# ansonb/RECON

Hardware: AMD Instinct MI355X
Metric: edges aggregated/sec (GAT fwd+bwd) on synthetic KG-context graphs (higher is better)
Workload: dtype f32

## Files before the change

### recon_amd/csrc/gat_atp.hip

```cpp
#include <math.h>
#include <stdlib.h>
#include "recon_common.h"

#include <type_traits>

namespace recon {
namespace {

constexpr int kBlock = 256;

__device__ __forceinline__ int xcd_block(int b, int nb) {
    const int q = nb >> 3, r = nb & 7, x = b & 7, i = b >> 3;
    return (x < r ? x * (q + 1) : r * (q + 1) + (x - r) * q) + i;
}
template <int VEC, bool B16>
__device__ __forceinline__ void load_in(float (&r)[VEC], const float* base, int64_t e) {
    if constexpr (!B16) {
        load_vec<VEC>(r, base + e);
    } else {
        const uint16_t* b = reinterpret_cast<const uint16_t*>(base) + e;
        if constexpr (VEC == 4) {
            const uint2 t = *reinterpret_cast<const uint2*>(b);
            r[0] = __builtin_bit_cast(float, t.x << 16); r[1] = __builtin_bit_cast(float, t.x & 0xffff0000u);
            r[2] = __builtin_bit_cast(float, t.y << 16); r[3] = __builtin_bit_cast(float, t.y & 0xffff0000u);
// ... 1948 lines not shown
    if (rc != RECON_OK) return rc;
    rc = recon_gat_atp_aggregate(g, a, stream);
    if (rc != RECON_OK) return rc;
    return recon_gat_atp_project(g, a, stream);
}

extern "C" int recon_gat_atp_bwd_gee_bf16_supported(int32_t F, int32_t R, int32_t D, int32_t H) {
    recon::AtpShape s;
    if (!recon_gat_atp_bf16_io_supported(F, R, D, H) || !recon::atp_shape(F, R, H, &s)) return 0;
    const size_t lds_k2 = static_cast<size_t>(H) * (F + R) * sizeof(float) + (kBlock / 64) * 512;
    const bool lring = s.vec == 4 && s.kr == 1 && lds_k2 + (kBlock / 64) * kK2LdsRingBytes <= 64 * 1024 && cfg_char(CFG_K2_LDS_RING) != '0';
    return (s.ht >= H && lring) ? 1 : 0;
}

extern "C" size_t recon_gat_atp_bwd_split_bytes(int32_t N, int32_t D, int32_t H) {
    if (N <= 0 || D <= 0 || H <= 0) return 256;
    return align_up(static_cast<size_t>(3) * N * bx3_kp(H * D) * 2, 256);
}

extern "C" size_t recon_gat_atp_bwd_partial_floats(int32_t N, int32_t E, int32_t F, int32_t R, int32_t D, int32_t H) {
    const int64_t W = 2LL * F + R;
    int s1 = gemm_pick_split_k(static_cast<int32_t>(W), D, N, H);
    const int s2 = bx3_kmajor_splits(N, bx3_kmajor_split_k(static_cast<int32_t>(W), D, N, H));
    if (s2 > s1) s1 = s2;
    size_t need = static_cast<size_t>(s1) * H * D * W;
    (void)E; (void)F; (void)R;
    return need > 0 ? need : 1;
}

constexpr int kSkinnySlices = 1024;
constexpr size_t kSkinnySrcLdsMax = 32 * 1024;
static int skinny_rpb(int64_t rows) {
    const int rpb = static_cast<int>(ceil_div64(rows, kSkinnySlices));
    return rpb < 32 ? 32 : rpb;
}
extern "C" size_t recon_gat_atp_bwd_partial2_floats(int32_t N, int32_t E, int32_t F, int32_t R, int32_t D, int32_t H) {
    (void)N; (void)E; (void)D; (void)H;
    const size_t mx = static_cast<size_t>(F > R ? F : R);
    return static_cast<size_t>(3) * kSkinnySlices * 16 * mx;
}
static int32_t skinny_red_blocks(int nj, int K) { return static_cast<int32_t>(ceil_div64(1LL * nj * K, 16)); }

extern "C" int recon_gat_atp_bwd_ride_plan(int32_t NR, int32_t N, int32_t E, int32_t F, int32_t R, int32_t D, int32_t H, int32_t* plan) {
    if (!plan || NR < 0 || N < 1 || E < 0 || F < 1 || R < 1 || D < 1 || H < 1) return 0;
    const int64_t rows[3] = {NR, N, E};
    const int K[3] = {F, F, R};
    int32_t nr_total = 0;
    for (int i = 0; i < 3; ++i) {
        plan[i] = rows[i] > 0 ? static_cast<int32_t>(ceil_div64(rows[i], skinny_rpb(rows[i]))) : 0;
        plan[3 + i] = rows[i] > 0 ? skinny_red_blocks(H, K[i]) : 0;
        nr_total += plan[3 + i];
    }
    const int32_t W = 2 * F + R;
    const int sk = bx3_kmajor_splits(NR, bx3_kmajor_split_k(W, D, NR, H));
    const int64_t tiles_xy = hx2_kmajor_tiles_xy(W, D);
    plan[6] = sk;
    plan[7] = static_cast<int32_t>(tiles_xy * H * sk);
    plan[8] = static_cast<int32_t>(1LL * H * sk + hx2_kmajor_rider_layers(tiles_xy, nr_total));
    plan[9] = nr_total;
    const bool lds_ok = static_cast<size_t>(skinny_rpb(N)) * H * sizeof(float) <= kSkinnySrcLdsMax;
    return (H <= 8 && D <= 256 && lds_ok && recon_gat_atp_f16x2_supported(F, R, D, H) && nr_total > 0) ? 1 : 0;
}

extern "C" int recon_gat_atp_bwd(const recon_graph* g, const recon_gat_atp_bwd_args* b, recon_stream_t stream) {
    return recon_gat_atp_bwd_phase(g, b, RECON_ATP_BWD_ALL, stream);
}

extern "C" int recon_gat_atp_bwd_phase(const recon_graph* g, const recon_gat_atp_bwd_args* b, int32_t phases, recon_stream_t stream) {
    if (!b) return RECON_ERR_INVALID;
    const recon_gat_atp_args* a = &b->fwd;
    int rc = check_atp(g, a);
    if (rc != RECON_OK) return rc;
    if (!recon_gat_atp_supported(a->N, a->E, a->F, a->R, a->D, a->H)) return RECON_ERR_UNSUPPORTED;
    if (!a->Z || !a->Zk || !b->grad_out || !b->g_V || !b->gxd || !b->Gs || !b->g_u || !b->partial || !b->partial2 || !b->q) return RECON_ERR_INVALID;
    if (a->E > 0 && (!a->sigma || !b->g_sigma || !b->Gxs)) return RECON_ERR_INVALID;
    const bool hx2 = atp_hx2(a);
    if ((a->concat || atp_rows(g, a).row_node) && !b->g_h && !hx2) return RECON_ERR_INVALID;
    if (hx2 && (!b->gh_split || (reinterpret_cast<uintptr_t>(b->gh_split) & 15) || (b->ld_gout & 3))) return RECON_ERR_INVALID;
    if (b->ld_gout < a->H * a->D) return RECON_ERR_INVALID;
    if (a->N == 0) return RECON_OK;
    hipStream_t st = as_stream(stream);
    const int32_t N = a->N, E = a->E, F = a->F, R = a->R, D = a->D, H = a->H, W = 2 * F + R;
    const AtpRows rw = atp_rows(g, a);
    const int32_t NR = rw.n;
    const int64_t HD = 1LL * H * D;
    AtpShape s;
    atp_shape(F, R, H, &s);
    const size_t lds_u = static_cast<size_t>(H) * (F + R) * sizeof(float);
    if (lds_u > 60 * 1024) return RECON_ERR_UNSUPPORTED;
    const size_t lds_k2 = lds_u + (kBlock / 64) * 512;

    const float* gh = b->grad_out;
    int32_t ld_gh = b->ld_gout;
    const int64_t ld_ghp = bx3_kp(static_cast<int32_t>(HD));
    const bool gh_planes = hx2 || (b->gh_split && a->a_split && !(reinterpret_cast<uintptr_t>(b->gh_split) & 15) && (D % 8) == 0 &&
                                   ((b->ld_gout | a->ld_out) & 3) == 0);
    uint16_t* ghp = gh_planes ? static_cast<uint16_t*>(b->gh_split) : nullptr;
    const int64_t ldi = (static_cast<int64_t>(NR) + 7) / 8 * 8;
    const size_t inv_off = align_up(static_cast<size_t>(2) * N * bx3_kp(static_cast<int32_t>(HD)) * 2, 256);
    const bool row_scaled = hx2 && D <= 256 && ((a->ld_out | b->ld_gout) & 3) == 0 && cfg_char(CFG_ATP_ROW_SCALE) != '0' &&
                            inv_off + static_cast<size_t>(H) * ldi * sizeof(float) <= recon_gat_atp_bwd_split_bytes(N, D, H);
    float* row_inv = row_scaled ? reinterpret_cast<float*>(static_cast<char*>(b->gh_split) + inv_off) : nullptr;
    if (phases & RECON_ATP_BWD_PREPARE) {
        if (hx2 && !row_scaled) {
            rc = hx2_amax(b->grad_out, N, static_cast<int32_t>(HD), b->ld_gout, atp_q(a, 3), st);
            if (rc != RECON_OK) return rc;
        }
// ... 108 lines not shown
                for (int i = 0; i < 3; ++i) {
                    sj[i] = SkinnyJob{nullptr, nullptr, nullptr, nullptr, 0, 0, 0, 0, 1, 0};
                    rj[i] = SkinnyRedJob{nullptr, nullptr, 0, 0, 0, 0, 0, 1, 0};
                    if (i >= count) continue;
                    const Prod& q = pr[i];
                    if (q.rows <= 0) {
                        for (int j = 0; j < q.nj; ++j) (void)hipMemsetAsync(q.out + (j % q.P) * q.S1 + (j / q.P) * q.S2, 0, sizeof(float) * q.K, st);
                        continue;
                    }
                    const int rpb = skinny_rpb(q.rows);
                    const int nb = static_cast<int>(ceil_div64(q.rows, rpb));
                    float* part = b->partial2 + i * third;
                    sj[i] = SkinnyJob{q.G, q.X, q.gather, part, q.ldg, q.nj, q.rows, q.K, rpb, nb};
                    rj[i] = SkinnyRedJob{part, q.out, q.S1, q.S2, nb, q.nj, q.K, q.P, skinny_red_blocks(q.nj, q.K)};
                    if (q.nj > nj_max) nj_max = q.nj;
                    nb_total += nb; nr_total += rj[i].nblocks;
                }
                if (share) { launch_src(); if (nb_total == 0) return; }
                else {
                    if (nb_total == 0) return;
                    const dim3 gp(static_cast<unsigned>(nb_total));
                    if (a->io_bf16) {
                        if (nj_max <= 8) hipLaunchKernelGGL((k_skinny_tn_partial<8, true>), gp, dim3(256), 0, st, sj[0], sj[1], sj[2]);
                        else hipLaunchKernelGGL((k_skinny_tn_partial<16, true>), gp, dim3(256), 0, st, sj[0], sj[1], sj[2]);
                    } else if (nj_max <= 8) hipLaunchKernelGGL((k_skinny_tn_partial<8>), gp, dim3(256), 0, st, sj[0], sj[1], sj[2]);
                    else hipLaunchKernelGGL((k_skinny_tn_partial<16>), gp, dim3(256), 0, st, sj[0], sj[1], sj[2]);
                }
                if (ride) { rider.j[0] = rj[0]; rider.j[1] = rj[1]; rider.j[2] = rj[2]; rider.nblocks = nr_total; }
                else hipLaunchKernelGGL(k_skinny_reduce, dim3(static_cast<unsigned>(nr_total)), dim3(1024), 0, st, rj[0], rj[1], rj[2]);
            };
            if (H <= 8) {
                const Prod pr[3] = {{b->Gs, 2 * H, H, a->x, rw.row_node, NR, F, H, W, 0, b->g_u},
                                    {b->Gs + H, 2 * H, H, a->x, nullptr, N, F, H, W, 0, b->g_u + F},
                                    {b->g_sigma, H, H, a->edge_embed, ee_gather, E, R, H, W, 0, b->g_u + 2 * F}};
                run_jobs(pr, 3);
            } else {
                for (int j = 0; j < 2 * H; ++j) {
                    const Prod one = {b->Gs + j, 2 * H, 1, a->x, j < H ? rw.row_node : nullptr, j < H ? NR : N, F, 1, W, 0,
                                      b->g_u + static_cast<int64_t>(j % H) * W + (j / H) * F};
                    run_jobs(&one, 1);
                }
                for (int h0 = 0; h0 < H; h0 += 16) {
                    const int nh = H - h0 < 16 ? H - h0 : 16;
                    const Prod one = {b->g_sigma + h0, H, nh, a->edge_embed, ee_gather, E, R, nh, W, 0, b->g_u + static_cast<int64_t>(h0) * W + 2 * F};
                    run_jobs(&one, 1);
                }
            }
        }
        RECON_CHECK_LAUNCH();
    }
    }
    if (b->g_a || b->g_a_2) {
        if (!b->g_a) return RECON_ERR_INVALID;
        if (phases & RECON_ATP_BWD_WEIGHTS) {
            OperandDesc A = plain_operand(a->V, static_cast<int64_t>(H) * W);
            OperandDesc B = plain_operand(gh, ld_gh);
            OutputDesc C = plain_output(b->g_a, W);
            GemmBatch bw = bt;
            bw.a_bs = W; bw.b_bs = D; bw.c_bs = static_cast<int64_t>(D) * W; bw.c_transpose = 1;
            const int64_t ldv = static_cast<int64_t>(H) * W;
            if (hx2) {
                const int sk = bx3_kmajor_splits(NR, bx3_kmajor_split_k(W, D, NR, H));
                rc = gemm_hx2_kmajor_batched(W, D, NR, a->V, 2LL * W, W, 2LL * NR * W, b->gh_split, 2LL * D, D, 2LL * NR * D,
                                             H, sk, b->partial, static_cast<const char*>(a->aux) + kHx2ZeroPageOffset, atp_scale_v(a), atp_scale_g(a), st,
                                             atp_dst_shared(a), row_inv, ldi, rider.nblocks > 0 ? &rider : nullptr);
                if (rc == RECON_OK && (phases & RECON_ATP_BWD_EARLY_SUM)) rc = splitk_reduce(b->partial, sk, W, D, C, bw.c_bs, H, 0, true, st);
            } else if (gh_planes && bx3_kmajor_supported(a->V, ldv, W, ld_ghp, D, W, D)) {
                const int sk = bx3_kmajor_splits(NR, bx3_kmajor_split_k(W, D, NR, H));
                rc = gemm_bx3_kmajor_batched(W, D, NR, a->V, ldv, W, b->gh_split, ld_ghp, static_cast<int64_t>(NR) * ld_ghp, D, H, sk, b->partial, st);
                if (rc == RECON_OK) rc = splitk_reduce(b->partial, sk, W, D, C, bw.c_bs, H, 0, true, st);
            } else {
                const int sk = gemm_pick_split_k(W, D, NR, H);
                rc = gemm_f32_batched(W, D, NR, A, false, B, false, C, bw, sk, b->partial, st);
            }
            if (rc != RECON_OK) return rc;
        }
        if ((phases & RECON_ATP_BWD_FINISH) && hx2 && !(phases & RECON_ATP_BWD_EARLY_SUM)) {
            const int sk = bx3_kmajor_splits(NR, bx3_kmajor_split_k(W, D, NR, H));
            const int ntile = static_cast<int>(ceil_div64(W, 32) * ceil_div64(D, 32)) * H;
            hipLaunchKernelGGL(k_atp_weights_finish, dim3(static_cast<unsigned>(ntile + ceil_div64(1LL * H * D, 8))), dim3(256), 0, st, b->partial, sk, W,
                               D, H, a->a, a->a_2, b->g_u, b->g_a, b->g_a_2, atp_q(a, 3), kHx2QuantityWords);
        } else if (phases & RECON_ATP_BWD_FINISH)
        hipLaunchKernelGGL(k_score_vec_bwd, dim3(static_cast<unsigned>(D), static_cast<unsigned>(H)), dim3(256), 0, st, a->a, a->a_2, b->g_u,
                           D, W, b->g_a, b->g_a_2, atp_hx2(a) ? atp_q(a, 3) : nullptr, kHx2QuantityWords);
        RECON_CHECK_LAUNCH();
    } else if ((phases & RECON_ATP_BWD_FINISH) && atp_hx2(a)) {
        if (hipMemsetAsync(atp_q(a, 3), 0, sizeof(uint32_t) * kHx2QuantityWords, st) != hipSuccess) return RECON_ERR_LAUNCH;
    }
    return RECON_OK;
}
```

### recon_amd/csrc/gemm_hx2.hip

```cpp
#include <stdlib.h>
#include "gemm_tile16.h"

namespace recon {
namespace {

constexpr int T = 2;

struct Hx2Args {
    const _Float16* Ap; const _Float16* Bp;
    int64_t a_plane, a_row, a_bs;
    int64_t b_plane, b_row, b_bs;
    OutputDesc C;
    int64_t c_bs;
    int32_t M, N, K;
    int32_t epilogue, c_vec4, xcd_remap, c_plain;
    int32_t a_shared_k;
    Hx2Scale sa, sb;
    const float* row_inv; int64_t row_inv_bs;
    int32_t a_span_bytes;
};

struct Hx2Terms {
    using V = f16x8;
    static constexpr int T = 2, NP = 3;
// ... 327 lines not shown
    bool b_rot[2];
#pragma unroll
    for (int hh = 0; hh < 2; ++hh) {
        const int k = 8 * g + 4 * hh + (ip >> 2);
#pragma unroll
        for (int i = 0; i < 2; ++i) a_off[i][hh] = k * 256 + (((2 * wid + i) ^ ka_h(k)) << 5) + ((ip & 3) << 3);
        b_row[hh] = k * (KB_SLOTS * 16) + (((ip & 3) & 1) << 3);
        b_rot[hh] = (k & 8) != 0;
    }
    auto b_off = [&](int j, int hh) { return b_row[hh] + (2 * j + ((ip & 3) >> 1) + (b_rot[hh] ? 2 : 0)) * 16; };
    float4 kin[2];
    float sg = 1.f;
    auto load_kinv = [&](int k0) {
        if constexpr (KSC) {
            const float* q = p.k_inv + bz * p.k_inv_bs + min(k0 + 8 * g, ((p.K + 7) & ~7) - 8);
            kin[0] = *reinterpret_cast<const float4*>(q);
            kin[1] = *reinterpret_cast<const float4*>(q + 4);
        }
    };
    auto mma_tile = [&]() {
        f16x8 a[2][T];
#pragma unroll
        for (int i = 0; i < 2; ++i)
#pragma unroll
            for (int q = 0; q < T; ++q) a[i][q] = tr_frag<f16x8>(As + q * KA_PLANE, a_off[i][0], a_off[i][1]);
        if constexpr (KSC) {
            const float f[8] = {kin[0].x, kin[0].y, kin[0].z, kin[0].w, kin[1].x, kin[1].y, kin[1].z, kin[1].w};
            f16x8 kf;
#pragma unroll
            for (int e = 0; e < 8; ++e) kf[e] = static_cast<_Float16>(fminf(f[e] * sg, 1.f));
#pragma unroll
            for (int i = 0; i < 2; ++i)
#pragma unroll
                for (int q = 0; q < T; ++q) a[i][q] = a[i][q] * kf;
        }
        mma_pairs<Hx2Terms>(acc, a, [&](int j, f16x8 (&dst)[T]) {
            const int o0 = b_off(j, 0), o1 = b_off(j, 1);
#pragma unroll
            for (int q = 0; q < T; ++q) dst[q] = tr_frag<f16x8>(Bs + q * KB_PLANE, o0, o1);
        });
    };

    if (k_begin < k_end) { dma(k_begin); load_kinv(k_begin); }
    const float ia = hx2_inv(hx2_scale_wave(p.sa));
    sg = hx2_scale_wave(p.sb);
    const float ib = hx2_inv(sg);
    for (int k0 = k_begin; k0 < k_end; k0 += BK) {
        asm volatile("s_waitcnt vmcnt(0)" ::: "memory");
        __syncthreads();
        mma_tile();
        __syncthreads();
        if (k0 + BK < k_end) { dma(k0 + BK); load_kinv(k0 + BK); }
    }
    float* base = p.partial + static_cast<int64_t>(tile.z) * p.M * p.N;
    const __amdgpu_buffer_rsrc_t rsrc = __builtin_amdgcn_make_buffer_rsrc(base, 0, p.M * p.N * 4, 0x00020000);
    const float sc = ia * ib;
#pragma unroll
    for (int i = 0; i < 2; ++i)
#pragma unroll
        for (int r = 0; r < 4; ++r) {
            const int row = m0 + mb + 16 * i + 4 * g + r;
            const int rowoff = row < p.M ? row * p.N : 0x1ffffff0;
#pragma unroll
            for (int j = 0; j < TN; ++j) {
                const int col = n0 + 16 * j + ip;
                const int off = col < p.N ? (rowoff + col) * 4 : 0x7ffffff0;
                __builtin_amdgcn_raw_buffer_store_b32(__builtin_bit_cast(uint32_t, acc[i][j][r] * sc), rsrc, off, 0, 0);
            }
        }
}

template <bool TRANS>
__global__ void __launch_bounds__(256) k_hx2_split_planes(const float* __restrict__ src, int64_t ld, int64_t src_bs, int32_t rows, int32_t K,
                                                          int32_t Kp, _Float16* __restrict__ dst, int64_t plane, int64_t dst_bs, const Hx2Scale sc) {
    const int64_t idx = static_cast<int64_t>(blockIdx.x) * 256 + threadIdx.x;
    const int kq = static_cast<int>(idx % (Kp / 8));
    const int r = static_cast<int>(idx / (Kp / 8));
    if (r >= rows) return;
    const float s = hx2_scale(sc);
    const float* sp = src + blockIdx.y * src_bs;
    float v[8];
#pragma unroll
    for (int j = 0; j < 8; ++j) {
        const int k = 8 * kq + j;
        v[j] = k < K ? (TRANS ? sp[static_cast<int64_t>(k) * ld + r] : sp[static_cast<int64_t>(r) * ld + k]) : 0.f;
    }
    uint32_t lo[4], hi[4];
#pragma unroll
    for (int j = 0; j < 4; ++j) hx2_split2(v[2 * j] * s, v[2 * j + 1] * s, lo[j], hi[j]);
    _Float16* d = dst + blockIdx.y * dst_bs + static_cast<int64_t>(r) * Kp + 8 * kq;
    *reinterpret_cast<u32x4*>(d) = u32x4{lo[0], lo[1], lo[2], lo[3]};
    *reinterpret_cast<u32x4*>(d + plane) = u32x4{hi[0], hi[1], hi[2], hi[3]};
}

__global__ void __launch_bounds__(256) k_hx2_split_both(const Hx2SplitBoth p) { hx2_split_both_block(p, blockIdx.x, blockIdx.y, blockIdx.z); }

template <int NTHREADS>
__global__ void __launch_bounds__(NTHREADS) k_hx2_amax(const float* __restrict__ src, int64_t rows, int32_t cols, int64_t ld, uint32_t* __restrict__ slot) {
    float m = 0.f;
    const int64_t stride = static_cast<int64_t>(gridDim.x) * NTHREADS;
    if (ld == cols && !(reinterpret_cast<uintptr_t>(src) & 15)) {
        const int64_t n = rows * cols, n4 = n >> 2;
        const float4* s4 = reinterpret_cast<const float4*>(src);
        int64_t i = static_cast<int64_t>(blockIdx.x) * NTHREADS + threadIdx.x;
        for (; i + 3 * stride < n4; i += 4 * stride) {
            const float4 v0 = s4[i], v1 = s4[i + stride], v2 = s4[i + 2 * stride], v3 = s4[i + 3 * stride];
// ... 72 lines not shown
    return RECON_OK;
}

bool hx2_supported(const void* Ap, int64_t a_plane, int64_t a_row, int64_t a_bs, int32_t K) {
    if (K <= 0 || (K & 7)) return false;
    return !((reinterpret_cast<uintptr_t>(Ap) & 15) || (a_plane & 7) || (a_row & 7) || (a_bs & 7));
}

int gemm_hx2_batched(int32_t M, int32_t N, int32_t K, const void* Ap, int64_t a_plane, int64_t a_row, int64_t a_bs, const void* Bplanes,
                     const OutputDesc& C, const GemmBatch& bt, const Hx2Scale& sa, const Hx2Scale& sb, hipStream_t st, int32_t a_shared_k,
                     const float* row_inv, int64_t row_inv_bs) {
    if (M < 0 || N < 0 || K < 0 || bt.batch < 0) return RECON_ERR_INVALID;
    if (M == 0 || N == 0 || bt.batch == 0) return RECON_OK;
    if (!Ap || !Bplanes || !C.base) return RECON_ERR_INVALID;
    if (!hx2_supported(Ap, a_plane, a_row, a_bs, K) || bt.c_transpose || bt.batch > 65535 || (reinterpret_cast<uintptr_t>(Bplanes) & 15))
        return RECON_ERR_UNSUPPORTED;
    Hx2Args a;
    a.Ap = static_cast<const _Float16*>(Ap); a.a_plane = a_plane; a.a_row = a_row; a.a_bs = a_bs;
    const int32_t Kp = hx2_kp(K);
    a.Bp = static_cast<const _Float16*>(Bplanes);
    a.b_row = Kp;
    a.b_bs = static_cast<int64_t>(N) * Kp;
    a.b_plane = a.b_bs * bt.batch;
    if (T * a.b_plane >= (1LL << 31)) return RECON_ERR_UNSUPPORTED;
    a.C = C; a.c_bs = bt.c_bs; a.M = M; a.N = N; a.K = K; a.epilogue = bt.epilogue;
    a.c_vec4 = c_vec4_ok(C, N, bt.c_bs) ? 1 : 0;
    a.xcd_remap = 1;
    if (a_shared_k < 0 || (a_shared_k & 7) || (a_shared_k && a_bs * bt.batch >= (1LL << 31))) return RECON_ERR_INVALID;
    a.a_shared_k = a_shared_k;
    a.c_plain = (a.c_vec4 && !C.scatter && C.P >= M && C.Dseg >= N && (static_cast<int64_t>(M) * C.S1 + N) * 4 < (1LL << 31)) ? 1 : 0;
    a.sa = sa; a.sb = sb;
    a.row_inv = row_inv; a.row_inv_bs = row_inv_bs;
    if (row_inv && sa.p0) return RECON_ERR_INVALID;
    const bool wide = K >= 1024 && ceil_div64(M, 256) * ceil_div64(N, BN) * bt.batch >= 256;
    const dim3 grid(static_cast<unsigned>(ceil_div64(N, BN)), static_cast<unsigned>(ceil_div64(M, wide ? 256 : BM)), static_cast<unsigned>(bt.batch));
    const int64_t a_span = ((T - 1) * a_plane + (bt.batch - 1) * a_bs + static_cast<int64_t>(M - 1) * a_row + hx2_kp(K) + 8) * 2;
    a.a_span_bytes = (a_plane >= 0 && a_bs >= 0 && a_row >= 0 && a_span < (1LL << 31) - 64) ? static_cast<int32_t>(a_span) : 0;
    const bool ring = !wide && a.a_span_bytes > 0 && cfg_char(CFG_HX2_RING) != '0';
    if (wide) hipLaunchKernelGGL((k_gemm_hx2<8>), grid, dim3(512), 0, st, a);
    else if (ring) hipLaunchKernelGGL((k_gemm_hx2_r3<4>), grid, dim3(NT), 0, st, a);
    else hipLaunchKernelGGL((k_gemm_hx2<4>), grid, dim3(NT), 0, st, a);
    if (hipGetLastError() != hipSuccess) return RECON_ERR_LAUNCH;
    return RECON_OK;
}

bool hx2_kmajor_supported(const void* Ap, int64_t lda, int64_t a_plane, int64_t a_bs, const void* Bp, int64_t ldb, int64_t b_plane,
                          int64_t b_bs, int32_t M, int32_t N) {
    const int64_t m_ld = (static_cast<int64_t>(M) + 7) / 8 * 8, n_ld = (static_cast<int64_t>(N) + 7) / 8 * 8;
    if (M < 1 || N < 1 || ((lda | a_plane | a_bs | ldb | b_plane | b_bs) & 7) || m_ld > lda || n_ld > ldb) return false;
    if (((M & 7) && a_bs != 0) || ((N & 7) && b_bs != 0)) return false;
    return !((reinterpret_cast<uintptr_t>(Ap) | reinterpret_cast<uintptr_t>(Bp)) & 15);
}

int64_t hx2_kmajor_tiles_xy(int32_t M, int32_t N) { return ceil_div64(N, BN) * ceil_div64(M, BM); }
int64_t hx2_kmajor_rider_layers(int64_t tiles_xy, int32_t rider_blocks) {
    return rider_blocks > 0 && tiles_xy > 0 ? ceil_div64(rider_blocks, tiles_xy) : 0;
}

int gemm_hx2_kmajor_batched(int32_t M, int32_t N, int32_t K, const void* Ap, int64_t lda, int64_t a_plane, int64_t a_bs, const void* Bp,
                            int64_t ldb, int64_t b_plane, int64_t b_bs, int32_t batch, int32_t split_k, float* partial, const void* zeros,
                            const Hx2Scale& sa, const Hx2Scale& sb, hipStream_t st, int32_t a_shared_m, const float* k_inv, int64_t k_inv_bs,
                            const SkinnyRedRider* rider) {
    if (M < 0 || N < 0 || K < 0 || batch < 0 || split_k < 1) return RECON_ERR_INVALID;
    const bool ride = rider && rider->nblocks > 0;
    if (ride && (M == 0 || N == 0 || batch == 0 || !k_inv)) return RECON_ERR_INVALID;
    if (M == 0 || N == 0 || batch == 0) return RECON_OK;
    if (!Ap || !Bp || !partial || !zeros || (reinterpret_cast<uintptr_t>(zeros) & 15)) return RECON_ERR_INVALID;
    if (!hx2_kmajor_supported(Ap, lda, a_plane, a_bs, Bp, ldb, b_plane, b_bs, M, N)) return RECON_ERR_UNSUPPORTED;
    Hx2KmArgs a;
    a.Ap = static_cast<const _Float16*>(Ap); a.Bp = static_cast<const _Float16*>(Bp); a.zeros = static_cast<const _Float16*>(zeros);
    a.lda = lda; a.ldb = ldb; a.a_plane = a_plane; a.b_plane = b_plane; a.a_bs = a_bs; a.b_bs = b_bs;
    a.partial = partial; a.M = M; a.N = N; a.K = K;
    a.m_ld = (M + 7) / 8 * 8; a.n_ld = (N + 7) / 8 * 8;
    const SplitK sp = splitk_plan(K, split_k);
    a.k_per_split = sp.k_per_split;
    a.nsplit = sp.nsplit;
    if (a.nsplit != split_k) return RECON_ERR_INVALID;
    a.tiles_z = batch * split_k;
    const int64_t gz = static_cast<int64_t>(a.tiles_z) + (ride ? hx2_kmajor_rider_layers(hx2_kmajor_tiles_xy(M, N), rider->nblocks) : 0);
    if (gz > 65535 || hx2_kmajor_tiles_xy(M, N) * gz >= (1LL << 31)) return RECON_ERR_UNSUPPORTED;
    a.sa = sa; a.sb = sb;
    if (a_shared_m < 0 || (a_shared_m & 7)) return RECON_ERR_UNSUPPORTED;
    a.a_shared_m = a_shared_m;
    const dim3 grid(static_cast<unsigned>(ceil_div64(N, BN)), static_cast<unsigned>(ceil_div64(M, BM)), static_cast<unsigned>(gz));
    a.k_inv = k_inv; a.k_inv_bs = k_inv_bs;
    if (k_inv && ((k_inv_bs & 3) || k_inv_bs < ((K + 7) & ~7) || (reinterpret_cast<uintptr_t>(k_inv) & 15))) return RECON_ERR_UNSUPPORTED;
    SkinnyRedRider none;
    none.nblocks = 0;
    for (SkinnyRedJob& j : none.j) j = SkinnyRedJob{nullptr, nullptr, 0, 0, 0, 0, 0, 1, 0};
    if (ride) hipLaunchKernelGGL((k_gemm_hx2_kmajor<2, true, true>), grid, dim3(NT), 0, st, a, *rider);
    else if (k_inv) hipLaunchKernelGGL((k_gemm_hx2_kmajor<2, true, false>), grid, dim3(NT), 0, st, a, none);
    else hipLaunchKernelGGL((k_gemm_hx2_kmajor<2, false, false>), grid, dim3(NT), 0, st, a, none);
    if (hipGetLastError() != hipSuccess) return RECON_ERR_LAUNCH;
    return RECON_OK;
}

}

static constexpr size_t kHdr = (recon::kHx2AuxBytes + 255) / 256 * 256;
extern "C" size_t recon_hx2_aux_bytes(void) { return recon::kHx2AuxBytes; }
static size_t hx2_planes_bytes(int64_t rows, int32_t K) { return align_up(static_cast<size_t>(2) * rows * recon::hx2_kp(K) * 2, 256); }

extern "C" size_t recon_sgemm_hx2_workspace_bytes(int32_t M, int32_t N, int32_t K) {
    if (M <= 0 || N <= 0 || K <= 0) return kHdr;
    return kHdr + hx2_planes_bytes(M, K) + hx2_planes_bytes(N, K);
}

extern "C" int recon_sgemm_hx2(int32_t M, int32_t N, int32_t K, const float* A, int32_t lda, const float* B, int32_t ldb, float* C_,
                               int32_t ldc, void* workspace, recon_stream_t stream) {
    using namespace recon;
    if (M < 0 || N < 0 || K < 0) return RECON_ERR_INVALID;
    if (M == 0 || N == 0) return RECON_OK;
    if (!A || !B || !C_ || !workspace || (reinterpret_cast<uintptr_t>(workspace) & 255)) return RECON_ERR_INVALID;
    if (K & 7) return RECON_ERR_UNSUPPORTED;
    hipStream_t st = as_stream(stream);
    char* ws = static_cast<char*>(workspace);
    uint32_t* slots = reinterpret_cast<uint32_t*>(ws);
    if (hipMemsetAsync(ws, 0, kHdr, st) != hipSuccess) return RECON_ERR_LAUNCH;
    int rc = hx2_amax(A, M, K, lda, slots + 0, st);
    if (rc == RECON_OK) rc = hx2_amax(B, N, K, ldb, slots + kHx2QuantityWords, st);
    if (rc != RECON_OK) return rc;
    const Hx2Scale sa{slots + 0, nullptr, 1.f}, sb{slots + kHx2QuantityWords, nullptr, 1.f};
    char* ap = ws + kHdr;
    char* bp = ap + hx2_planes_bytes(M, K);
    rc = hx2_split_planes(A, lda, 0, false, M, K, 1, ap, sa, st);
    if (rc == RECON_OK) rc = hx2_split_planes(B, ldb, 0, false, N, K, 1, bp, sb, st);
    if (rc != RECON_OK) return rc;
    GemmBatch bt;
    bt.batch = 1; bt.a_bs = bt.b_bs = bt.c_bs = 0; bt.epilogue = GEMM_EPI_NONE;
    const int64_t Kp = hx2_kp(K);
    return gemm_hx2_batched(M, N, K, ap, static_cast<int64_t>(M) * Kp, Kp, 0, bp, plain_output(C_, ldc), bt, sa, sb, st);
}

extern "C" int recon_sgemm_hx2_presplit(int32_t M, int32_t N, int32_t K, float* C_, int32_t ldc, void* workspace, recon_stream_t stream) {
    using namespace recon;
    if (M <= 0 || N <= 0 || K <= 0 || (K & 7) || !C_ || !workspace) return RECON_ERR_INVALID;
    char* ws = static_cast<char*>(workspace);
    uint32_t* slots = reinterpret_cast<uint32_t*>(ws);
    const Hx2Scale sa{slots + 0, nullptr, 1.f}, sb{slots + kHx2QuantityWords, nullptr, 1.f};
    char* ap = ws + kHdr;
    char* bp = ap + hx2_planes_bytes(M, K);
    GemmBatch bt;
    bt.batch = 1; bt.a_bs = bt.b_bs = bt.c_bs = 0; bt.epilogue = GEMM_EPI_NONE;
    const int64_t Kp = hx2_kp(K);
    return gemm_hx2_batched(M, N, K, ap, static_cast<int64_t>(M) * Kp, Kp, 0, bp, plain_output(C_, ldc), bt, sa, sb, as_stream(stream));
}

extern "C" size_t recon_sgemm_hx2_tn_workspace_bytes(int32_t M, int32_t N, int32_t K) {
    using namespace recon;
    if (M <= 0 || N <= 0 || K <= 0) return kHdr;
    const int sk = bx3_kmajor_splits(K, bx3_kmajor_split_k(M, N, K, 1));
    return kHdr + hx2_planes_bytes(K, M) + hx2_planes_bytes(K, N) + static_cast<size_t>(sk) * M * N * sizeof(float) + 256;
}

static int hx2_tn(int32_t M, int32_t N, int32_t K, const float* A, int32_t lda, const float* B, int32_t ldb, float* C_, int32_t ldc,
                  void* workspace, bool split, recon_stream_t stream) {
    using namespace recon;
    if (M < 0 || N < 0 || K < 0) return RECON_ERR_INVALID;
    if (M == 0 || N == 0) return RECON_OK;
    if (!C_ || !workspace || (reinterpret_cast<uintptr_t>(workspace) & 255)) return RECON_ERR_INVALID;
    hipStream_t st = as_stream(stream);
    char* ws = static_cast<char*>(workspace);
    uint32_t* slots = reinterpret_cast<uint32_t*>(ws);
    const Hx2Scale sa{slots + 0, nullptr, 1.f}, sb{slots + kHx2QuantityWords, nullptr, 1.f};
    char* ap = ws + kHdr;
    char* bp = ap + hx2_planes_bytes(K, M);
    float* partial = reinterpret_cast<float*>(bp + hx2_planes_bytes(K, N));
    const int64_t Mp = hx2_kp(M), Np = hx2_kp(N);
    int rc = RECON_OK;
    if (split) {
        if (!A || !B) return RECON_ERR_INVALID;
        if (hipMemsetAsync(ws, 0, kHdr, st) != hipSuccess) return RECON_ERR_LAUNCH;
        rc = hx2_amax(A, K, M, lda, slots + 0, st);
        if (rc == RECON_OK) rc = hx2_amax(B, K, N, ldb, slots + kHx2QuantityWords, st);
        if (rc == RECON_OK) rc = hx2_split_planes(A, lda, 0, false, K, M, 1, ap, sa, st);
        if (rc == RECON_OK) rc = hx2_split_planes(B, ldb, 0, false, K, N, 1, bp, sb, st);
        if (rc != RECON_OK) return rc;
    }
    const int sk = bx3_kmajor_splits(K, bx3_kmajor_split_k(M, N, K, 1));
    rc = gemm_hx2_kmajor_batched(M, N, K, ap, Mp, static_cast<int64_t>(K) * Mp, 0, bp, Np, static_cast<int64_t>(K) * Np, 0, 1, sk, partial,
                                 ws + kHx2ZeroPageOffset, sa, sb, st);
    if (rc != RECON_OK) return rc;
    return splitk_reduce(partial, sk, M, N, plain_output(C_, ldc), 0, 1, GEMM_EPI_NONE, false, st);
}

extern "C" int recon_sgemm_hx2_tn(int32_t M, int32_t N, int32_t K, const float* A, int32_t lda, const float* B, int32_t ldb, float* C_,
                                  int32_t ldc, void* workspace, recon_stream_t stream) {
    return hx2_tn(M, N, K, A, lda, B, ldb, C_, ldc, workspace, true, stream);
}
extern "C" int recon_sgemm_hx2_tn_presplit(int32_t M, int32_t N, int32_t K, float* C_, int32_t ldc, void* workspace, recon_stream_t stream) {
    return hx2_tn(M, N, K, nullptr, 0, nullptr, 0, C_, ldc, workspace, false, stream);
}
```

### recon_amd/csrc/gemm_tile16.h

```cpp
#pragma once
#include "gemm_common.h"

namespace recon {

constexpr int BM = 128, BN = 208, BK = 32, NT = 256, TN = 13;
using bf16x8 = __attribute__((ext_vector_type(8))) __bf16;
using f16x8 = __attribute__((ext_vector_type(8))) _Float16;
using f32x4 = __attribute__((ext_vector_type(4))) float;
using u32x4 = __attribute__((ext_vector_type(4))) uint32_t;
using i16x4 = __attribute__((ext_vector_type(4))) short;

constexpr int B_PLANE = BN * 64;
constexpr int KB_SLOTS = 28;
constexpr int KA_PLANE = BK * 256, KB_PLANE = BK * KB_SLOTS * 16;


__device__ __forceinline__ int lds_off(int row, int kq) { return row * 64 + (((kq + 2 * (row >> 3)) & 3) << 4); }

template <int T>
__device__ __forceinline__ int b_image_src(int slot, int n0, int N, int64_t b_plane, int64_t b_row) {
    const int s = min(slot, T * B_PLANE / 16 - 1);
    const int plane = T == 1 ? 0 : s / (BN * 4), rem = T == 1 ? s : s % (BN * 4), rowL = rem >> 2, pslot = rem & 3;
    const int kq = (pslot - 2 * (rowL >> 3)) & 3;
    const int j = rowL >> 4, rho = rowL & 15;
// ... 35 lines not shown
                        *reinterpret_cast<float4*>(crow + minor_off(C.Dseg, C.Sseg, col)) =
                            make_float4(fin(acc[i][4 * q][r]), fin(acc[i][4 * q + 1][r]), fin(acc[i][4 * q + 2][r]), fin(acc[i][4 * q + 3][r]));
                } else {
#pragma unroll
                    for (int jj = 0; jj < 4; ++jj)
                        if (col + jj < N) crow[minor_off(C.Dseg, C.Sseg, col + jj)] = fin(acc[i][4 * q + jj][r]);
                }
            }
            const int col = n0 + 192 + li;
            if (col < N) crow[minor_off(C.Dseg, C.Sseg, col)] = fin(acc[i][12][r]);
        }
}


template <class S, int NJ>
__device__ __forceinline__ void products(f32x4 (&acc)[2][TN], const typename S::V (&a)[2][S::T], const typename S::V (&b)[2][S::T], int j0) {
#pragma unroll
    for (int t = 0; t < S::NP; ++t)
#pragma unroll
        for (int jj = 0; jj < NJ; ++jj)
#pragma unroll
            for (int i = 0; i < 2; ++i) acc[i][j0 + jj] = S::mfma(t, a[i], b[jj], acc[i][j0 + jj]);
}

template <class S, class Read>
__device__ __forceinline__ void mma_pairs(f32x4 (&acc)[2][TN], const typename S::V (&a)[2][S::T], Read read) {
    typename S::V b[2][2][S::T];
    auto read_pair = [&](int j0, typename S::V (&dst)[2][S::T]) {
#pragma unroll
        for (int jj = 0; jj < 2; ++jj)
            if (j0 + jj < TN) read(j0 + jj, dst[jj]);
    };
    read_pair(0, b[0]);
#pragma unroll
    for (int g = 0; g < (TN + 1) / 2; ++g) {
        if (2 * g + 2 < TN) read_pair(2 * g + 2, b[(g + 1) & 1]);
        __builtin_amdgcn_sched_barrier(0);
        if (2 * g + 1 < TN) products<S, 2>(acc, a, b[g & 1], 2 * g);
        else products<S, 1>(acc, a, b[g & 1], 2 * g);
        __builtin_amdgcn_sched_barrier(0);
    }
}


__device__ __forceinline__ int ka_h(int k) { return (k & 3) | (((k >> 3) & 1) << 2); }

template <class V>
__device__ __forceinline__ V tr_frag(const unsigned char* base, int off_lo, int off_hi) {
    const i16x4 lo = __builtin_amdgcn_ds_read_tr16_b64_v4i16((__attribute__((address_space(3))) i16x4*)(base + off_lo));
    const i16x4 hi = __builtin_amdgcn_ds_read_tr16_b64_v4i16((__attribute__((address_space(3))) i16x4*)(base + off_hi));
    return __builtin_bit_cast(V, __builtin_shufflevector(lo, hi, 0, 1, 2, 3, 4, 5, 6, 7));
}


inline int32_t tile_kp(int32_t K) { return (K + BK - 1) / BK * BK; }

struct SplitK { int32_t k_per_split, nsplit; };
inline SplitK splitk_plan(int32_t K, int32_t split_k) {
    int64_t kps = ceil_div64(K > 0 ? K : 1, split_k);
    kps = ceil_div64(kps, BK) * BK;
    return {static_cast<int32_t>(kps), static_cast<int32_t>(ceil_div64(K > 0 ? K : 1, kps))};
}

inline bool c_vec4_ok(const OutputDesc& C, int32_t N, int64_t c_bs) {
    return !(N & 3) && !(c_bs & 3) && !(reinterpret_cast<uintptr_t>(C.base) & 15) && !(C.S1 & 3) && !(C.S2 & 3) && !(C.Sseg & 3) &&
           (C.Dseg >= N || !(C.Dseg & 3));
}

}
```

### recon_amd/csrc/recon_common.h

```cpp
#pragma once
#include <hip/hip_runtime.h>
#include <stdint.h>
#include "recon_hip.h"

#define RECON_CHECK_LAUNCH()                                   \
    do {                                                       \
        if (hipGetLastError() != hipSuccess) return RECON_ERR_LAUNCH; \
    } while (0)

static inline hipStream_t as_stream(recon_stream_t s) { return reinterpret_cast<hipStream_t>(s); }
static inline int64_t ceil_div64(int64_t a, int64_t b) { return (a + b - 1) / b; }
static inline size_t align_up(size_t x, size_t a) { return (x + a - 1) / a * a; }

namespace recon {

constexpr int kWave = 64;

enum CfgKey { CFG_GCN_FUSED, CFG_GCN_FUSED_BWD, CFG_GEMM_CFG, CFG_GEMM_LIN, CFG_GEMM_SPLITK, CFG_GEMM_XCD, CFG_PROP_B16, CFG_PROP_B16_YPOST,
              CFG_PROP_BWD, CFG_PROP_BWD_CHAIN, CFG_PROP_BWD_WIDE, CFG_PROP_FWD, CFG_PROP_LDS_KB, CFG_ATP_ROW_SCALE, CFG_GRAPH_SMALL, CFG_KG_NHOP,
              CFG_HX2_RING, CFG_K2_LDS_RING, CFG_K2_PERSIST, CFG_COUNT };
const char* cfg(CfgKey k);
int cfg_int(CfgKey k, int dflt);
char cfg_char(CfgKey k);
int32_t* nan_flag();
// ... 285 lines not shown
bool hx2_kmajor_supported(const void* Ap, int64_t lda, int64_t a_plane, int64_t a_bs, const void* Bp, int64_t ldb, int64_t b_plane,
                          int64_t b_bs, int32_t M, int32_t N);

struct SkinnyRedJob { const float* partial; float* out; int64_t S1, S2; int32_t nb, nj, K, P, nblocks; };
struct SkinnyRedRider { SkinnyRedJob j[3]; int32_t nblocks; };
template <int NT>
__device__ __forceinline__ void skinny_reduce_block(const SkinnyRedJob& j0, const SkinnyRedJob& j1, const SkinnyRedJob& j2, int blk, int tid,
                                                    float (*red)[17]) {
    static_assert(NT == 1024 || NT == 256, "64 slice groups x 16 elements over the block");
    constexpr int GPT = 1024 / NT, GSTEP = NT / 16;
    const int which = blk < j0.nblocks ? 0 : (blk < j0.nblocks + j1.nblocks ? 1 : 2);
    const SkinnyRedJob& jb = which == 0 ? j0 : (which == 1 ? j1 : j2);
    const float* __restrict__ partial = jb.partial;
    const int nb = jb.nb, tot = jb.nj * jb.K;
    const int bid = blk - (which == 0 ? 0 : (which == 1 ? j0.nblocks : j0.nblocks + j1.nblocks));
    const int e = tid & 15, g0 = tid >> 4;
    const int idx = bid * 16 + e;
    const int idc = min(idx, tot - 1);
    const int per = (nb + 63) / 64;
    float s[GPT][4];
    int b0[GPT], len[GPT];
#pragma unroll
    for (int i = 0; i < GPT; ++i) {
        b0[i] = (g0 + i * GSTEP) * per;
        len[i] = max(0, min(nb, b0[i] + per) - b0[i]);
        s[i][0] = s[i][1] = s[i][2] = s[i][3] = 0.f;
    }
    for (int k = 0; k < per; k += 4) {
        float v[GPT][4];
#pragma unroll
        for (int i = 0; i < GPT; ++i)
#pragma unroll
            for (int q = 0; q < 4; ++q) v[i][q] = partial[static_cast<int64_t>(min(b0[i] + k + q, nb - 1)) * tot + idc];
#pragma unroll
        for (int i = 0; i < GPT; ++i) {
            const bool quad = k + 4 <= len[i];
#pragma unroll
            for (int q = 0; q < 4; ++q) s[i][q] = quad ? s[i][q] + v[i][q] : s[i][q];
#pragma unroll
            for (int q = 0; q < 4; ++q) s[i][0] = (!quad && k + q < len[i]) ? s[i][0] + v[i][q] : s[i][0];
        }
    }
#pragma unroll
    for (int i = 0; i < GPT; ++i) red[g0 + i * GSTEP][e] = (s[i][0] + s[i][1]) + (s[i][2] + s[i][3]);
    __syncthreads();
    if (g0 == 0 && idx < tot) {
        float t = 0.f;
#pragma unroll
        for (int g = 0; g < 64; ++g) t += red[g][e];
        const int j = idx / jb.K, c = idx % jb.K;
        jb.out[(j % jb.P) * jb.S1 + (j / jb.P) * jb.S2 + c] = t;
    }
}
int64_t hx2_kmajor_tiles_xy(int32_t M, int32_t N);
int64_t hx2_kmajor_rider_layers(int64_t tiles_xy, int32_t rider_blocks);
int gemm_hx2_kmajor_batched(int32_t M, int32_t N, int32_t K, const void* Ap, int64_t lda, int64_t a_plane, int64_t a_bs, const void* Bp,
                            int64_t ldb, int64_t b_plane, int64_t b_bs, int32_t batch, int32_t split_k, float* partial, const void* zeros,
                            const Hx2Scale& sa, const Hx2Scale& sb, hipStream_t st, int32_t a_shared_m = 0, const float* k_inv = nullptr,
                            int64_t k_inv_bs = 0, const SkinnyRedRider* rider = nullptr);
int splitk_reduce(const float* partial, int32_t splits, int32_t M, int32_t N, const OutputDesc& C, int64_t c_bs, int32_t batch,
                  int32_t epilogue, bool transpose, hipStream_t st);

}
```

Before: 82.52 million.

## Add 256-row wide-tile k-major hx2 GEMM kernel for standalone TN sgemm path

```diff
diff --git a/recon_amd/csrc/gat_atp.hip b/recon_amd/csrc/gat_atp.hip
--- a/recon_amd/csrc/gat_atp.hip
+++ b/recon_amd/csrc/gat_atp.hip
@@ -2024,7 +2024,7 @@
         nr_total += plan[3 + i];
     }
     const int32_t W = 2 * F + R;
-    const int sk = bx3_kmajor_splits(NR, bx3_kmajor_split_k(W, D, NR, H));
+    const int sk = bx3_kmajor_splits(NR, hx2_kmajor_split_k(W, D, NR, H, false));
     const int64_t tiles_xy = hx2_kmajor_tiles_xy(W, D);
     plan[6] = sk;
     plan[7] = static_cast<int32_t>(tiles_xy * H * sk);
@@ -2239,6 +2239,7 @@
     }
     if (b->g_a || b->g_a_2) {
         if (!b->g_a) return RECON_ERR_INVALID;
+        const int sk_hx2 = hx2 ? bx3_kmajor_splits(NR, hx2_kmajor_split_k(W, D, NR, H, false)) : 1;
         if (phases & RECON_ATP_BWD_WEIGHTS) {
             OperandDesc A = plain_operand(a->V, static_cast<int64_t>(H) * W);
             OperandDesc B = plain_operand(gh, ld_gh);
@@ -2247,7 +2248,7 @@
             bw.a_bs = W; bw.b_bs = D; bw.c_bs = static_cast<int64_t>(D) * W; bw.c_transpose = 1;
             const int64_t ldv = static_cast<int64_t>(H) * W;
             if (hx2) {
-                const int sk = bx3_kmajor_splits(NR, bx3_kmajor_split_k(W, D, NR, H));
+                const int sk = sk_hx2;
                 rc = gemm_hx2_kmajor_batched(W, D, NR, a->V, 2LL * W, W, 2LL * NR * W, b->gh_split, 2LL * D, D, 2LL * NR * D,
                                              H, sk, b->partial, static_cast<const char*>(a->aux) + kHx2ZeroPageOffset, atp_scale_v(a), atp_scale_g(a), st,
                                              atp_dst_shared(a), row_inv, ldi, rider.nblocks > 0 ? &rider : nullptr);
@@ -2263,7 +2264,7 @@
             if (rc != RECON_OK) return rc;
         }
         if ((phases & RECON_ATP_BWD_FINISH) && hx2 && !(phases & RECON_ATP_BWD_EARLY_SUM)) {
-            const int sk = bx3_kmajor_splits(NR, bx3_kmajor_split_k(W, D, NR, H));
+            const int sk = sk_hx2;
             const int ntile = static_cast<int>(ceil_div64(W, 32) * ceil_div64(D, 32)) * H;
             hipLaunchKernelGGL(k_atp_weights_finish, dim3(static_cast<unsigned>(ntile + ceil_div64(1LL * H * D, 8))), dim3(256), 0, st, b->partial, sk, W,
                                D, H, a->a, a->a_2, b->g_u, b->g_a, b->g_a_2, atp_q(a, 3), kHx2QuantityWords);
diff --git a/recon_amd/csrc/gemm_hx2.hip b/recon_amd/csrc/gemm_hx2.hip
--- a/recon_amd/csrc/gemm_hx2.hip
+++ b/recon_amd/csrc/gemm_hx2.hip
@@ -403,6 +403,164 @@
         __syncthreads();
         if (k0 + BK < k_end) { dma(k0 + BK); load_kinv(k0 + BK); }
     }
+    float* base = p.partial + static_cast<int64_t>(tile.z) * p.M * p.N;
+    const __amdgpu_buffer_rsrc_t rsrc = __builtin_amdgcn_make_buffer_rsrc(base, 0, p.M * p.N * 4, 0x00020000);
+    const float sc = ia * ib;
+#pragma unroll
+    for (int i = 0; i < 2; ++i)
+#pragma unroll
+        for (int r = 0; r < 4; ++r) {
+            const int row = m0 + mb + 16 * i + 4 * g + r;
+            const int rowoff = row < p.M ? row * p.N : 0x1ffffff0;
+#pragma unroll
+            for (int j = 0; j < TN; ++j) {
+                const int col = n0 + 16 * j + ip;
+                const int off = col < p.N ? (rowoff + col) * 4 : 0x7ffffff0;
+                __builtin_amdgcn_raw_buffer_store_b32(__builtin_bit_cast(uint32_t, acc[i][j][r] * sc), rsrc, off, 0, 0);
+            }
+        }
+}
+
+constexpr int KA256_PIECES = T * (KA256_PLANE / 1024), KA256_DMA = KA256_PIECES / 8;
+constexpr int KB256_DMA = (KB_PIECES + 7) / 8;
+constexpr int KM256_A_RING = 3, KM256_A_STAGE = T * KA256_PLANE, KM256_B_STAGE = T * KB_PLANE;
+constexpr int KM256_B_AT = KM256_A_RING * KM256_A_STAGE, KM256_SCRATCH_AT = KM256_B_AT + 2 * KM256_B_STAGE;
+constexpr int KM256_LDS = KM256_SCRATCH_AT + 1024;
+
+__global__ void __launch_bounds__(512, 1) k_gemm_hx2_kmajor256(const Hx2KmArgs p) {
+    __shared__ __attribute__((aligned(16))) unsigned char S[KM256_LDS];
+    unsigned char* const scratch = S + KM256_SCRATCH_AT;
+    const int t = threadIdx.x, lane = t & 63;
+    const int wid = __builtin_amdgcn_readfirstlane(t >> 6);
+    const TileId tile = xcd_tile(1);
+    const int m0 = tile.y * BM256, n0 = tile.x * BN;
+    const int bz = tile.z / p.nsplit, zs = tile.z % p.nsplit;
+    const int k_begin = zs * p.k_per_split, k_end = min(p.K, k_begin + p.k_per_split);
+    const int KT = k_begin < k_end ? (k_end - k_begin + BK - 1) / BK : 0;
+
+    const _Float16* pa[KA256_DMA];
+    const _Float16* pb[KB256_DMA];
+    int a_k[KA256_DMA], b_k[KB256_DMA];
+#pragma unroll
+    for (int i = 0; i < KA256_DMA; ++i) {
+        const int pc = 8 * i + wid, s = 64 * (pc & 15) + lane;
+        a_k[i] = k_begin + (s >> 5);
+        int64_t col = min(m0 + ka256_src_col(s), p.m_ld - 8);
+        if (col >= p.a_shared_m) col += bz * p.a_bs;
+        pa[i] = p.Ap + (pc >> 4) * p.a_plane + static_cast<int64_t>(a_k[i]) * p.lda + col;
+    }
+#pragma unroll
+    for (int i = 0; i < KB256_DMA; ++i) {
+        const int pc = min(8 * i + wid, KB_PIECES - 1);
+        const int s = 64 * (pc % (KB_PIECES / T)) + lane, k = s / KB_SLOTS, phys = s % KB_SLOTS;
+        int slot = phys - ((k & 8) ? 2 : 0);
+        if (slot < 0 || slot >= 26) slot = 0;
+        b_k[i] = k_begin + k;
+        pb[i] = p.Bp + bz * p.b_bs + (pc / (KB_PIECES / T)) * p.b_plane + static_cast<int64_t>(b_k[i]) * p.ldb + min(n0 + 8 * slot, p.n_ld - 8);
+    }
+    const _Float16* zlane = p.zeros + 8 * lane;
+    const int64_t a_step = static_cast<int64_t>(BK) * p.lda, b_step = static_cast<int64_t>(BK) * p.ldb;
+    int ka_adv = 0, kb_adv = 0;
+    auto dma_a = [&](int stage) {
+        const bool real = k_begin + ka_adv < k_end;
+        unsigned char* const st = S + stage * KM256_A_STAGE;
+#pragma unroll
+        for (int i = 0; i < KA256_DMA; ++i) {
+            const int pc = 8 * i + wid;
+            dma16_to_lds(a_k[i] + ka_adv < k_end ? pa[i] : zlane, real ? st + (pc >> 4) * KA256_PLANE + 1024 * (pc & 15) : scratch);
+            pa[i] += a_step;
+        }
+        ka_adv += BK;
+    };
+    auto dma_b = [&](int stage) {
+        const bool real = k_begin + kb_adv < k_end;
+        unsigned char* const st = S + KM256_B_AT + stage * KM256_B_STAGE;
+#pragma unroll
+        for (int i = 0; i < KB256_DMA; ++i) {
+            const int pc = 8 * i + wid;
+            const bool piece = real && pc < KB_PIECES;
+            dma16_to_lds(b_k[i] + kb_adv < k_end ? pb[i] : zlane, piece ? st + (pc / (KB_PIECES / T)) * KB_PLANE + 1024 * (pc % (KB_PIECES / T)) : scratch);
+            pb[i] += b_step;
+        }
+        kb_adv += BK;
+    };
+
+    f32x4 acc[2][TN];
+#pragma unroll
+    for (int i = 0; i < 2; ++i)
+#pragma unroll
+        for (int j = 0; j < TN; ++j) acc[i][j] = f32x4{0.f, 0.f, 0.f, 0.f};
+
+    const int mb = wid * 32;
+    const int ip = lane & 15, g = lane >> 4;
+    int a_off[2][2], b_base[2];
+#pragma unroll
+    for (int hh = 0; hh < 2; ++hh) {
+        const int k = 8 * g + 4 * hh + (ip >> 2);
+#pragma unroll
+        for (int i = 0; i < 2; ++i) a_off[i][hh] = ka256_off(k, 2 * wid + i, ip);
+        b_base[hh] = k * (KB_SLOTS * 16) + (((ip & 3) & 1) << 3) + ((((ip & 3) >> 1) + ((k & 8) ? 2 : 0)) << 4);
+    }
+    int sa = 0, par = 0;
+    auto step = [&]() {
+        dma_wait<KA256_DMA>();
+        __builtin_amdgcn_s_barrier();
+        asm volatile("" ::: "memory");
+        const unsigned char* At = S + sa * KM256_A_STAGE;
+        const unsigned char* Bt = S + KM256_B_AT + par * KM256_B_STAGE;
+        const int sa_free = sa == 0 ? KM256_A_RING - 1 : sa - 1;
+        sa = sa + 1 == KM256_A_RING ? 0 : sa + 1;
+        par ^= 1;
+        f16x8 a[2][T];
+#pragma unroll
+        for (int i = 0; i < 2; ++i)
+#pragma unroll
+            for (int q = 0; q < T; ++q) a[i][q] = tr_frag<f16x8>(At + q * KA256_PLANE, a_off[i][0], a_off[i][1]);
+        f16x8 b[2][2][T];
+        auto read_pair = [&](int j0, f16x8 (&dst)[2][T]) {
+#pragma unroll
+            for (int jj = 0; jj < 2; ++jj)
+                if (j0 + jj < TN) {
+#pragma unroll
+                    for (int q = 0; q < T; ++q) dst[jj][q] = tr_frag<f16x8>(Bt + q * KB_PLANE, b_base[0] + (j0 + jj) * 32, b_base[1] + (j0 + jj) * 32);
+                }
+        };
+        read_pair(0, b[0]);
+#pragma unroll
+        for (int gq = 0; gq < (TN + 1) / 2; ++gq) {
+            if (2 * gq + 2 < TN) read_pair(2 * gq + 2, b[(gq + 1) & 1]);
+            __builtin_amdgcn_sched_barrier(0);
+            if (2 * gq + 1 < TN) products<Hx2Terms, 2>(acc, a, b[gq & 1], 2 * gq);
+            else products<Hx2Terms, 1>(acc, a, b[gq & 1], 2 * gq);
+            __builtin_amdgcn_sched_barrier(0);
+            if (gq == 0) {
+                dma_b(par);
+                dma_a(sa_free);
+                __builtin_amdgcn_sched_barrier(0);
+            }
+        }
+    };
+
+    dma_a(0);
+    dma_b(0);
+    dma_a(1);
+    const float ia = hx2_inv(hx2_scale_wave(p.sa)), ib = hx2_inv(hx2_scale_wave(p.sb));
+    const bool live = m0 + mb < p.M;
+    if (live) {
+#pragma unroll 1
+        for (int kt = 0; kt < KT; ++kt) step();
+    } else {
+#pragma unroll 1
+        for (int kt = 0; kt < KT; ++kt) {
+            dma_wait<KA256_DMA>();
+            __builtin_amdgcn_s_barrier();
+            asm volatile("" ::: "memory");
+            dma_b((kt + 1) & 1);
+            dma_a((kt + 2) % KM256_A_RING);
+        }
+    }
+    dma_wait<0>();
+    if (!live) return;
     float* base = p.partial + static_cast<int64_t>(tile.z) * p.M * p.N;
     const __amdgpu_buffer_rsrc_t rsrc = __builtin_amdgcn_make_buffer_rsrc(base, 0, p.M * p.N * 4, 0x00020000);
     const float sc = ia * ib;
@@ -581,7 +739,16 @@
     return !((reinterpret_cast<uintptr_t>(Ap) | reinterpret_cast<uintptr_t>(Bp)) & 15);
 }
 
-int64_t hx2_kmajor_tiles_xy(int32_t M, int32_t N) { return ceil_div64(N, BN) * ceil_div64(M, BM); }
+bool hx2_kmajor_wide(int32_t M, bool wide) { return wide && M > BM; }
+int64_t hx2_kmajor_tiles_xy(int32_t M, int32_t N, bool wide) { return ceil_div64(N, BN) * ceil_div64(M, hx2_kmajor_wide(M, wide) ? BM256 : BM); }
+int hx2_kmajor_split_k(int32_t M, int32_t N, int32_t K, int32_t batch, bool wide) {
+    if (!hx2_kmajor_wide(M, wide)) return bx3_kmajor_split_k(M, N, K, batch);
+    const int64_t tiles = hx2_kmajor_tiles_xy(M, N, true) * (batch > 0 ? batch : 1);
+    int64_t s = 256 / (tiles > 0 ? tiles : 1);
+    if (s > K / (4 * BK)) s = K / (4 * BK);
+    if (s > 64) s = 64;
+    return static_cast<int>(s < 1 ? 1 : s);
+}
 int64_t hx2_kmajor_rider_layers(int64_t tiles_xy, int32_t rider_blocks) {
     return rider_blocks > 0 && tiles_xy > 0 ? ceil_div64(rider_blocks, tiles_xy) : 0;
 }
@@ -589,7 +756,7 @@
 int gemm_hx2_kmajor_batched(int32_t M, int32_t N, int32_t K, const void* Ap, int64_t lda, int64_t a_plane, int64_t a_bs, const void* Bp,
                             int64_t ldb, int64_t b_plane, int64_t b_bs, int32_t batch, int32_t split_k, float* partial, const void* zeros,
                             const Hx2Scale& sa, const Hx2Scale& sb, hipStream_t st, int32_t a_shared_m, const float* k_inv, int64_t k_inv_bs,
-                            const SkinnyRedRider* rider) {
+                            const SkinnyRedRider* rider, bool want_wide) {
     if (M < 0 || N < 0 || K < 0 || batch < 0 || split_k < 1) return RECON_ERR_INVALID;
     const bool ride = rider && rider->nblocks > 0;
     if (ride && (M == 0 || N == 0 || batch == 0 || !k_inv)) return RECON_ERR_INVALID;
@@ -606,18 +773,21 @@
     a.nsplit = sp.nsplit;
     if (a.nsplit != split_k) return RECON_ERR_INVALID;
     a.tiles_z = batch * split_k;
-    const int64_t gz = static_cast<int64_t>(a.tiles_z) + (ride ? hx2_kmajor_rider_layers(hx2_kmajor_tiles_xy(M, N), rider->nblocks) : 0);
-    if (gz > 65535 || hx2_kmajor_tiles_xy(M, N) * gz >= (1LL << 31)) return RECON_ERR_UNSUPPORTED;
+    const int64_t gz = static_cast<int64_t>(a.tiles_z) + (ride ? hx2_kmajor_rider_layers(hx2_kmajor_tiles_xy(M, N, want_wide), rider->nblocks) : 0);
+    if (gz > 65535 || hx2_kmajor_tiles_xy(M, N, want_wide) * gz >= (1LL << 31)) return RECON_ERR_UNSUPPORTED;
     a.sa = sa; a.sb = sb;
     if (a_shared_m < 0 || (a_shared_m & 7)) return RECON_ERR_UNSUPPORTED;
     a.a_shared_m = a_shared_m;
-    const dim3 grid(static_cast<unsigned>(ceil_div64(N, BN)), static_cast<unsigned>(ceil_div64(M, BM)), static_cast<unsigned>(gz));
+    const bool wide = hx2_kmajor_wide(M, want_wide);
+    if (wide && (ride || k_inv)) return RECON_ERR_UNSUPPORTED;
+    const dim3 grid(static_cast<unsigned>(ceil_div64(N, BN)), static_cast<unsigned>(ceil_div64(M, wide ? BM256 : BM)), static_cast<unsigned>(gz));
     a.k_inv = k_inv; a.k_inv_bs = k_inv_bs;
     if (k_inv && ((k_inv_bs & 3) || k_inv_bs < ((K + 7) & ~7) || (reinterpret_cast<uintptr_t>(k_inv) & 15))) return RECON_ERR_UNSUPPORTED;
     SkinnyRedRider none;
     none.nblocks = 0;
     for (SkinnyRedJob& j : none.j) j = SkinnyRedJob{nullptr, nullptr, 0, 0, 0, 0, 0, 1, 0};
-    if (ride) hipLaunchKernelGGL((k_gemm_hx2_kmajor<2, true, true>), grid, dim3(NT), 0, st, a, *rider);
+    if (wide) hipLaunchKernelGGL(k_gemm_hx2_kmajor256, grid, dim3(512), 0, st, a);
+    else if (ride) hipLaunchKernelGGL((k_gemm_hx2_kmajor<2, true, true>), grid, dim3(NT), 0, st, a, *rider);
     else if (k_inv) hipLaunchKernelGGL((k_gemm_hx2_kmajor<2, true, false>), grid, dim3(NT), 0, st, a, none);
     else hipLaunchKernelGGL((k_gemm_hx2_kmajor<2, false, false>), grid, dim3(NT), 0, st, a, none);
     if (hipGetLastError() != hipSuccess) return RECON_ERR_LAUNCH;
@@ -678,7 +848,7 @@
 extern "C" size_t recon_sgemm_hx2_tn_workspace_bytes(int32_t M, int32_t N, int32_t K) {
     using namespace recon;
     if (M <= 0 || N <= 0 || K <= 0) return kHdr;
-    const int sk = bx3_kmajor_splits(K, bx3_kmajor_split_k(M, N, K, 1));
+    const int sk = bx3_kmajor_splits(K, hx2_kmajor_split_k(M, N, K, 1, true));
     return kHdr + hx2_planes_bytes(K, M) + hx2_planes_bytes(K, N) + static_cast<size_t>(sk) * M * N * sizeof(float) + 256;
 }
 
@@ -706,9 +876,9 @@
         if (rc == RECON_OK) rc = hx2_split_planes(B, ldb, 0, false, K, N, 1, bp, sb, st);
         if (rc != RECON_OK) return rc;
     }
-    const int sk = bx3_kmajor_splits(K, bx3_kmajor_split_k(M, N, K, 1));
+    const int sk = bx3_kmajor_splits(K, hx2_kmajor_split_k(M, N, K, 1, true));
     rc = gemm_hx2_kmajor_batched(M, N, K, ap, Mp, static_cast<int64_t>(K) * Mp, 0, bp, Np, static_cast<int64_t>(K) * Np, 0, 1, sk, partial,
-                                 ws + kHx2ZeroPageOffset, sa, sb, st);
+                                 ws + kHx2ZeroPageOffset, sa, sb, st, 0, nullptr, 0, nullptr, true);
     if (rc != RECON_OK) return rc;
     return splitk_reduce(partial, sk, M, N, plain_output(C_, ldc), 0, 1, GEMM_EPI_NONE, false, st);
 }
diff --git a/recon_amd/csrc/gemm_tile16.h b/recon_amd/csrc/gemm_tile16.h
--- a/recon_amd/csrc/gemm_tile16.h
+++ b/recon_amd/csrc/gemm_tile16.h
@@ -111,6 +111,14 @@
     return __builtin_bit_cast(V, __builtin_shufflevector(lo, hi, 0, 1, 2, 3, 4, 5, 6, 7));
 }
 
+constexpr int BM256 = 256;
+constexpr int KA256_PLANE = BK * 512;
+__device__ __forceinline__ int ka256_off(int k, int chunk, int ip) { return k * 512 + ((chunk ^ ka_h(k)) << 5) + ((ip & 3) << 3); }
+__device__ __forceinline__ int ka256_src_col(int s) {
+    const int k = s >> 5, phys = s & 31;
+    return 16 * ((phys >> 1) ^ ka_h(k)) + 8 * (phys & 1);
+}
+
 
 inline int32_t tile_kp(int32_t K) { return (K + BK - 1) / BK * BK; }
 
diff --git a/recon_amd/csrc/recon_common.h b/recon_amd/csrc/recon_common.h
--- a/recon_amd/csrc/recon_common.h
+++ b/recon_amd/csrc/recon_common.h
@@ -361,12 +361,14 @@
         jb.out[(j % jb.P) * jb.S1 + (j / jb.P) * jb.S2 + c] = t;
     }
 }
-int64_t hx2_kmajor_tiles_xy(int32_t M, int32_t N);
+bool hx2_kmajor_wide(int32_t M, bool wide);
+int hx2_kmajor_split_k(int32_t M, int32_t N, int32_t K, int32_t batch, bool wide);
+int64_t hx2_kmajor_tiles_xy(int32_t M, int32_t N, bool wide = false);
 int64_t hx2_kmajor_rider_layers(int64_t tiles_xy, int32_t rider_blocks);
 int gemm_hx2_kmajor_batched(int32_t M, int32_t N, int32_t K, const void* Ap, int64_t lda, int64_t a_plane, int64_t a_bs, const void* Bp,
                             int64_t ldb, int64_t b_plane, int64_t b_bs, int32_t batch, int32_t split_k, float* partial, const void* zeros,
                             const Hx2Scale& sa, const Hx2Scale& sb, hipStream_t st, int32_t a_shared_m = 0, const float* k_inv = nullptr,
-                            int64_t k_inv_bs = 0, const SkinnyRedRider* rider = nullptr);
+                            int64_t k_inv_bs = 0, const SkinnyRedRider* rider = nullptr, bool want_wide = false);
 int splitk_reduce(const float* partial, int32_t splits, int32_t M, int32_t N, const OutputDesc& C, int64_t c_bs, int32_t batch,
                   int32_t epilogue, bool transpose, hipStream_t st);
 
```

After: 81.67 million. 0.99x the previous value.
